# buwantaiji/FermiFlow

Hardware: AMD Instinct MI355X
Metric: walker-steps/sec (full VMC iteration: 100 MCMC steps + generate + E_loc + grad + Adam) (higher is better)
Workload: dtype f64

## Files before the change

fermiflow_amd/csrc/ff_cnf_adj.hip:

```cpp
#include "ff_common.h"
#include "ff_ode.h"
#include "ff_radial.h"

#ifdef FF_STAMPS
#define FF_STAMP(i) do { unsigned long long t_ = __builtin_amdgcn_s_memtime(); stamp_acc[i] += t_ - stamp_prev; stamp_prev = t_; } while (0)
#else
#define FF_STAMP(i) do { } while (0)
#endif

struct ff_adj_args {
  int64_t B;
  ff_net net;
  double ta, tb, rtol, atol;
  int max_steps;
  const double* z_in;
  const double* az_in;
  const double* ad_in;
  const double* w_e;
  const double* w_mean;
  const int32_t* w_index;
  double w_scale;
  double* gx_out;
  double* rows;
  double* trows;
  double* off_table;
  int32_t* stats;
  const double* h_init;
  double h_scale;
  int h_equal;
  double* h_out;
  int32_t* wcost;
  const int32_t* order;
  int unit0;
};

template <int N, int D, int MAXU>
__global__ void __launch_bounds__(FF_WAVE)
ff_ode_adj_kernel(ff_adj_args A) {
  using Gm = ff_geom<N, D>;
  constexpr int M = Gm::M, G = Gm::G, P = Gm::P, R = Gm::RA;
  constexpr int NV = 2;
  {
    const double* rt = A.net.radial_table;
    if (rt && rt[3] == 0.0 && rt[4] == 0.0 && *A.off_table == 0.0) return;
  }

  __shared__ ff_wtab s_w[2][FF_HPAD];
  __shared__ double s_z[G][M], s_kb[G][M], s_err[G][M], s_ad[G];
  __shared__ double s_rad[G][R], s_rinv[G][R], s_ca[G][R], s_cb[G][R];
  constexpr int CH = 8;
  __shared__ double s_ph[G][M][CH][3], s_hd[G][R][3];
  __shared__ int s_pa[R], s_pb[R], s_any;
  __shared__ double s_e2[64];

  __shared__ int s_st[4];
#include "ff_adj_direct_body.inc"
}

template <int N, int D>
struct ff_adj_smem {
  static constexpr int M = ff_geom<N, D>::M, G = ff_geom<N, D>::G, R = ff_geom<N, D>::RA, CH = 8;
  ff_wtab s_w[2][FF_HPAD];
  double s_z[G][M], s_kb[G][M], s_err[G][M], s_ad[G];
  double s_rad[G][R], s_rinv[G][R], s_ca[G][R], s_cb[G][R];
  double s_ph[G][M][CH][3], s_hd[G][R][3];
  double s_e2[64];
  int s_pa[R], s_pb[R], s_any, s_st[4];
};

template <int N, int D, int MAXU>
__global__ void __launch_bounds__(FF_WAVE, 4)
ff_ode_adj_lean_kernel(ff_adj_args A) {
  using Gm = ff_geom<N, D>;
  constexpr int M = Gm::M, G = Gm::G, P = Gm::P, R = Gm::RA;
  constexpr int NV = 2;
  {
    const double* rt = A.net.radial_table;
    if (rt && rt[3] == 0.0 && rt[4] == 0.0 && *A.off_table == 0.0) return;
  }
  FF_DYN_LDS(ff_adj_lean_lds);
  ff_adj_smem<N, D>& sm = *reinterpret_cast<ff_adj_smem<N, D>*>(ff_adj_lean_lds);
  auto& s_w = sm.s_w; auto& s_z = sm.s_z; auto& s_kb = sm.s_kb; auto& s_err = sm.s_err; auto& s_ad = sm.s_ad;
  auto& s_rad = sm.s_rad; auto& s_rinv = sm.s_rinv; auto& s_ca = sm.s_ca; auto& s_cb = sm.s_cb;
  constexpr int CH = ff_adj_smem<N, D>::CH;
  auto& s_ph = sm.s_ph; auto& s_hd = sm.s_hd; auto& s_pa = sm.s_pa; auto& s_pb = sm.s_pb; auto& s_any = sm.s_any;
  auto& s_e2 = sm.s_e2; auto& s_st = sm.s_st;
#include "ff_adj_direct_body.inc"
}

struct ff_rec { double dr, ca, cb; int j; };
#define FF_DEP_LROW (FF_DEP_ROW + 1)

FF_D void ff_row_add(double (*sW)[FF_DEP_NLDS][FF_DEP_LROW], double* __restrict__ ovf, int t, int j, const double* c, int nrow) {
  if (j < FF_DEP_NLDS) {
    double* row = &sW[t][j][0];
#pragma unroll
    for (int k = 0; k < 6; k++) atomicAdd(row + k, c[k]);
#pragma unroll
    for (int k0 = 6; k0 < FF_DEP_ROW; k0 += 2) {
      if (nrow > k0) { atomicAdd(row + k0, c[k0]); atomicAdd(row + k0 + 1, c[k0 + 1]); }
    }
  } else {
    double* row = ovf + ((size_t)t * FF_DEP_NTOT + j) * FF_DEP_ROW;
#pragma unroll
    for (int k = 0; k < FF_DEP_ROW; k++) atomicAdd(row + k, c[k]);
    int jo = j;
    FF_OPAQUE(jo);
  }
}

FF_D void ff_deposit(double (*sW)[FF_DEP_NLDS][FF_DEP_LROW], double* __restrict__ ovf, int t, const ff_rec& rc, double w, int nrow) {
  if (w == 0.0) return;
  double pk = 1.0, pm = 0.0, c[FF_DEP_ROW];
#pragma unroll
  for (int k = 0; k < FF_DEP_ROW; k++) {
    c[k] = w * fma(rc.ca, pk, rc.cb * pm);
    pm = pk;
    pk = pk * rc.dr * (1.0 / (k + 1));
  }
  ff_row_add(sW, ovf, t, rc.j, c, nrow);
}

FF_D void ff_deposit5(double (*sW)[FF_DEP_NLDS][FF_DEP_LROW], double* __restrict__ ovf, int t, const ff_rec& q0, const ff_rec& q2,
                      const ff_rec& q3, const ff_rec& q4, const ff_rec& q5, double hw, int nrow) {
  if (hw == 0.0) return;
  const ff_rec* rc[5] = {&q0, &q2, &q3, &q4, &q5};
  const double bw[5] = {hw * FF_B0, hw * FF_B2, hw * FF_B3, hw * FF_B4, hw * FF_B5};
  constexpr double HD = 1.0 / FF_DEP_INVH;
  double rm = 0.0;
#pragma unroll
  for (int e = 0; e < 5; e++) rm += fma((double)rc[e]->j, HD, rc[e]->dr);
  double jcf = rint(rm * (0.2 * FF_DEP_INVH));
  jcf = fmin(fmax(jcf, 0.0), (double)(FF_DEP_NTOT - 1));
  const int jC = (rm == rm) ? (int)jcf : 0;
  double acc[FF_DEP_ROW];
#pragma unroll
  for (int k = 0; k < FF_DEP_ROW; k++) acc[k] = 0.0;
#pragma unroll
  for (int e = 0; e < 5; e++) {
    const double dr = fma((double)(rc[e]->j - jC), HD, rc[e]->dr);
    if (fabs(dr) <= 1.5 * HD) {
      double pk = bw[e], pm = 0.0;
#pragma unroll
      for (int k = 0; k < FF_DEP_ROW; k++) {
        acc[k] += fma(rc[e]->ca, pk, rc[e]->cb * pm);
        pm = pk;
        pk = pk * dr * (1.0 / (k + 1));
      }
    } else {
      ff_deposit(sW, ovf, t, *rc[e], bw[e], nrow);
    }
  }
  ff_row_add(sW, ovf, t, jC, acc, nrow);
}

#ifndef FF_ADJ_WPS
#define FF_ADJ_WPS 1
#endif
#ifndef FF_ADJ_WPW
#define FF_ADJ_WPW 2
#endif
#ifndef FF_ADJ_G12
#define FF_ADJ_G12 3
#endif
constexpr int ff_adjtab_G(int n, int d) {
  const int M = n * d;
  if (M <= 0 || M > FF_WAVE) return 0;
  const int g = FF_WAVE / M > 16 ? 16 : FF_WAVE / M;
  if (M == 12) return FF_ADJ_G12;
  if (d == 2 && (n == 4 || n == 5 || n == 7 || n == 9 || n == 10 || n == 11)) {
    const int gr = FF_WAVE / (n * (n + 1) / 2);
    return gr < 1 ? 1 : (gr < g ? gr : g);
  }
  return g;
}
template <int N, int D> struct ff_adjtab_geom { static constexpr int G = ff_adjtab_G(N, D); };
static int adj_tab_G(int n, int d) { return ff_adjtab_G(n, d); }

template <int N, int D, int WPW>
__global__ void __launch_bounds__(FF_WAVE * WPW, WPW > 1 ? WPW : FF_ADJ_WPS)
ff_ode_adjtab_kernel(ff_adj_args A) {
  using Gm = ff_geom<N, D>;
  constexpr int M = Gm::M, G = ff_adjtab_geom<N, D>::G, P = Gm::P, R = Gm::RA;
  constexpr int NV = 2, NSLOT = (G * R + FF_WAVE - 1) / FF_WAVE;
#ifdef FF_PRIO_ADJTAB
  FF_SETPRIO();
#endif
  const double* __restrict__ rtab = A.net.radial_table;
  if (!(rtab && rtab[3] == 0.0 && rtab[4] == 0.0)) return;
  const int dep_nrow = FF_UNIFORM(rtab[5] >= 6.0 && rtab[5] <= (double)FF_DEP_ROW ? (int)rtab[5] : FF_DEP_ROW);

  __shared__ double s_z_[WPW][G][M], s_kb_[WPW][G][M], s_err_[WPW][G][M], s_ad_[WPW][G], s_hw_[WPW][G];
  constexpr int TROW = N * 3 * D + 1;
  __shared__ double s_T_[WPW][G][N][TROW];
  __shared__ double s_W[2][FF_DEP_NLDS][FF_DEP_LROW];
  __shared__ int s_pa[R], s_pb[R], s_any_[WPW];
  __shared__ int s_turn, s_done[2];

  const int wv = WPW > 1 ? (int)(threadIdx.x >> 6) : 0, lane = threadIdx.x & (FF_WAVE - 1);
  auto& s_z = s_z_[wv]; auto& s_kb = s_kb_[wv]; auto& s_err = s_err_[wv]; auto& s_ad = s_ad_[wv]; auto& s_hw = s_hw_[wv];
  auto& s_T = s_T_[wv]; int& s_any = s_any_[wv];
  const int g = lane / M, i = lane % M;
  const bool ingrp = g < G;
  const int gg = ingrp ? g : 0;
  const int ai = i / D, ci = i % D;
  for (int e = threadIdx.x; e < 2 * FF_DEP_NLDS * FF_DEP_LROW; e += FF_WAVE * WPW) (&s_W[0][0][0])[e] = 0.0;
  if (threadIdx.x == 0) {
    int p = 0;
    for (int a = 0; a < N; a++)
      for (int b = a + 1; b < N; b++) { s_pa[p] = a; s_pb[p] = b; p++; }
    for (int a = 0; a < N; a++) { if (P + a < R) { s_pa[P + a] = a; s_pb[P + a] = -1; } }
    s_turn = 0; s_done[0] = 0; s_done[1] = 0;
  }
  __syncthreads();
  const int He = A.net.He, Hm = A.net.Hm;
  const bool has_mu = Hm > 0;
  const int nrad = has_mu ? (P + N) : P;
  const double tab_inv_h = rtab[0], tab_h = rtab[1];
  const double rtol = A.rtol, atol = A.atol;
  int rq_id[NSLOT];
#pragma unroll
  for (int sl = 0; sl < NSLOT; sl++) {
    const int q = lane + sl * FF_WAVE;
    const bool act = q < G * nrad;
    const int qg = act ? q / nrad : 0, p = act ? q - qg * nrad : 0;
    rq_id[sl] = act ? (qg | (s_pa[p] << 4) | ((s_pb[p] < 0 ? 15 : s_pb[p]) << 8) | (p << 12)) : -1;
  }
  bool off_any = false;
  constexpr double NT = 2 * M;
  const int64_t ngroups = (A.B + G - 1) / G;
  __shared__ int s_st[4];
  if (threadIdx.x < 4) s_st[threadIdx.x] = 0;
  int my_turn = wv;
  double* const ovf = A.trows + (size_t)gridDim.x * 2 * FF_DEP_NLDS * FF_DEP_ROW;
#ifdef FF_STAMPS
  unsigned long long stamp_acc[9] = {0, 0, 0, 0, 0, 0, 0, 0, 0}, stamp_prev = __builtin_amdgcn_s_memtime();
#endif

  for (int64_t grp = (int64_t)blockIdx.x * WPW + wv; grp < ngroups; grp += (int64_t)gridDim.x * WPW) {
    const int64_t bq = grp * G + g;
    const bool valid = ingrp && bq < A.B;
    const int64_t b = ff_opt_load(A.order, valid, bq, A.z_in, (int32_t)bq);
    double y[NV], k0[NV] = {0.0, 0.0}, k1[NV] = {0.0, 0.0}, k2[NV] = {0.0, 0.0}, k3[NV] = {0.0, 0.0}, k4[NV] = {0.0, 0.0}, k5[NV] = {0.0, 0.0};
    y[0] = ff_opt_load(A.z_in, valid, b * M + i, A.z_in, 0.25 * (i + 1) + 0.125 * ((i * 7) % 5));
    {
      const bool ws = A.w_e != nullptr;
      const int wi = ff_opt_load(A.w_index, valid && ws, b, A.z_in, (int32_t)0);
      const double wb = (ff_opt_load(A.w_e, valid, b, A.z_in, 0.0) - ff_opt_load(A.w_mean, valid && ws, wi, A.z_in, 0.0)) * A.w_scale;
      const double az0 = ff_opt_load(A.az_in, valid, b * M + i, A.z_in, 0.0), ad0 = ff_opt_load(A.ad_in, valid, b, A.z_in, 0.0);
      y[1] = ws ? wb * az0 : az0;
      if (ingrp && i == 0) s_ad[g] = ws ? -wb : ad0;
    }
    ff_rec r0[NSLOT], r2[NSLOT], r3[NSLOT], r4[NSLOT], r5[NSLOT], r6[NSLOT];
    ff_stepper S;
    S.begin(A.ta, A.tb, valid);
    const double hwarm = ff_open_step(ff_opt_load(A.h_init, valid, A.h_scale < 0.0 ? 0 : b, A.z_in, 0.0) * fabs(A.h_scale), A.ta, A.tb, A.h_equal);
    const bool warm = hwarm > 0.0;
    double hmax_acc = 0.0;
    int s = -2, nev = 0;
    double h0v = 0.0, d1v = 0.0;

    auto group_sum = [&](double part) -> double {
      if (ingrp) s_err[g][i] = part;
      FF_WAVE_ORDER();
      double t = 0.0;
#pragma unroll
      for (int j = 0; j < M; j++) t += s_err[gg][j];
      FF_WAVE_ORDER();
      return t;
    };

    auto evaluate = [&](auto stage_tag) -> bool {
      constexpr int SG = decltype(stage_tag)::value;
      if constexpr (SG == FF_STAGE_DYN) FF_ASSUME(s <= 0);
      const int sv = SG == FF_STAGE_DYN ? s : SG;
      double in[NV];
      const double h = S.h;
      {
        const double hsel = (sv == -1) ? h0v * S.dir : h;
#pragma unroll
        for (int v = 0; v < NV; v++) in[v] = y[v];
        switch (sv) {
          case -1:
#pragma unroll
            for (int v = 0; v < NV; v++) in[v] = fma(hsel, k0[v], y[v]);
            break;
          case 1:
#pragma unroll
            for (int v = 0; v < NV; v++) in[v] = fma(hsel * FF_A10, k0[v], y[v]);
            break;
          case 2:
#pragma unroll
            for (int v = 0; v < NV; v++) in[v] = fma(hsel * FF_A21, k1[v], fma(hsel * FF_A20, k0[v], y[v]));
            break;
          case 3:
#pragma unroll
            for (int v = 0; v < NV; v++) in[v] = fma(hsel * FF_A32, k2[v], fma(hsel * FF_A31, k1[v], fma(hsel * FF_A30, k0[v], y[v])));
            break;
          case 4:
#pragma unroll
            for (int v = 0; v < NV; v++)
              in[v] = fma(hsel * FF_A43, k3[v], fma(hsel * FF_A42, k2[v], fma(hsel * FF_A41, k1[v], fma(hsel * FF_A40, k0[v], y[v]))));
            break;
          case 5:
#pragma unroll
            for (int v = 0; v < NV; v++)
              in[v] = fma(hsel * FF_A54, k4[v], fma(hsel * FF_A53, k3[v], fma(hsel * FF_A52, k2[v], fma(hsel * FF_A51, k1[v], fma(hsel * FF_A50, k0[v], y[v])))));
            break;
          case 6:
#pragma unroll
            for (int v = 0; v < NV; v++)
              in[v] = fma(hsel * FF_B5, k5[v], fma(hsel * FF_B4, k4[v], fma(hsel * FF_B3, k3[v], fma(hsel * FF_B2, k2[v], fma(hsel * FF_B0, k0[v], y[v])))));
            break;
          default: break;
        }
      }
      FF_STAMP(0);
      FF_WAVE_ORDER();
      if (ingrp) { s_z[g][i] = in[0]; s_kb[g][i] = in[1]; }
      FF_WAVE_ORDER();
      FF_STAMP(1);
      ff_rec cur[NSLOT];
      double rq_rho[NSLOT][D], rq_dl[NSLOT][D], rq_r[NSLOT], rq_ri[NSLOT], rq_T[NSLOT][3 + 5], rq_dr[NSLOT];
      bool rq_ok[NSLOT];
#pragma unroll
      for (int sl = 0; sl < NSLOT; sl++) {
        const int id = rq_id[sl];
        const bool act = id >= 0;
        const int qg = act ? (id & 15) : 0, a = act ? ((id >> 4) & 15) : 0, bq = act ? ((id >> 8) & 15) : 15;
        const bool pair = bq != 15;
        const int bb = pair ? bq : a;
        double r2 = 0.0;
#pragma unroll
        for (int c = 0; c < D; c++) {
          rq_rho[sl][c] = s_z[qg][a * D + c] - (pair ? s_z[qg][bb * D + c] : 0.0);
          rq_dl[sl][c] = s_kb[qg][a * D + c] - (pair ? s_kb[qg][bb * D + c] : 0.0);
          r2 = fma(rq_rho[sl][c], rq_rho[sl][c], r2);
        }
        ff_sqrt_rcp(r2, rq_r[sl], rq_ri[sl]);
        rq_dr[sl] = 0.0;
        rq_ok[sl] = ff_table_fetch<3>(rtab, tab_inv_h, tab_h, pair ? 0 : 1, rq_r[sl], rq_T[sl], rq_dr[sl]);
      }
#pragma unroll
      for (int sl = 0; sl < NSLOT; sl++) {
        const int id = rq_id[sl];
        cur[sl].j = 0; cur[sl].dr = 0.0; cur[sl].ca = 0.0; cur[sl].cb = 0.0;
        if (id >= 0) {
          const int qg = id & 15, a = (id >> 4) & 15, bq = (id >> 8) & 15;
          const bool pair = bq != 15;
          const int bb = pair ? bq : a;
          const double* rho = rq_rho[sl];
          const double* dl = rq_dl[sl];
          const double r = rq_r[sl], ri = rq_ri[sl], ad = s_ad[qg];
          double hd[3] = {0.0, 0.0, 0.0}, al = 0.0;
          if (rq_ok[sl]) ff_table_eval<3>(rq_T[sl], rq_dr[sl], hd);
#pragma unroll
          for (int c = 0; c < D; c++) al = fma(dl[c], rho[c], al);
          double jf = rint(r * FF_DEP_INVH);
          if ((!rq_ok[sl] || !(jf <= (double)(FF_DEP_NTOT - 1))) && (grp * G + qg) < A.B) off_any = true;
          jf = fmin(jf, (double)(FF_DEP_NTOT - 1));
          cur[sl].j = (r == r) ? (int)jf : 0;
          cur[sl].dr = fma(-jf, 1.0 / FF_DEP_INVH, r);
          cur[sl].ca = pair ? -(al - 2.0 * D * ad) : -(al - D * ad);
          cur[sl].cb = pair ? 2.0 * ad * r : ad * r;
          const double f0 = hd[0], f1 = hd[1], f2 = hd[2];
          const double F1 = f1 * (al * ri), gq = (pair ? 2.0 : 1.0) * fma(f2, r, (1.0 + D) * f1) * ri;
          double* Ta = &s_T[qg][a][bb * 3 * D];
#pragma unroll
          for (int c = 0; c < D; c++) {
            const double pv = f0 * rho[c], pw = fma(F1, rho[c], f0 * dl[c]), pg = gq * rho[c];
            Ta[c] = pv; Ta[D + c] = pw; Ta[2 * D + c] = pg;
          }
        }
      }
      FF_WAVE_ORDER();
      nev++;
      FF_STAMP(2);
      double out[NV];
      {
        double vi = 0.0, dvk = 0.0, gdi = 0.0;
#pragma unroll
        for (int j = 0; j < N; j++) {
          const bool use = has_mu || j != ai;
          const bool lower = j < ai;
          const double* T = lower ? &s_T[gg][j][ai * 3 * D + ci] : &s_T[gg][ai][j * 3 * D + ci];
          const double sg = lower ? -1.0 : 1.0;
          const double tv = T[0], tw = T[D], tg = T[2 * D];
          vi = fma(sg, use ? tv : 0.0, vi); dvk = fma(sg, use ? tw : 0.0, dvk); gdi = fma(sg, use ? tg : 0.0, gdi);
        }
        out[0] = vi;
        out[1] = fma(s_ad[gg], gdi, -dvk);
      }
      FF_STAMP(3);
      const int s_before = sv;
      if (sv == -2) {
#pragma unroll
        for (int v = 0; v < NV; v++) k0[v] = out[v];
#pragma unroll
        for (int sl = 0; sl < NSLOT; sl++) r0[sl] = cur[sl];
        double p0 = 0.0, p1 = 0.0;
#pragma unroll
        for (int v = 0; v < NV; v++) {
          const double isc = ff_rcp(fma(fabs(y[v]), rtol, atol));
          p0 = fma(y[v] * isc, y[v] * isc, p0);
          p1 = fma(k0[v] * isc, k0[v] * isc, p1);
        }
        const double d0 = sqrt(group_sum(p0) * (1.0 / NT));
        d1v = sqrt(group_sum(p1) * (1.0 / NT));
        h0v = S.h0(d0, d1v);
        s = -1;
        if (!ff_wave_or_w(&s_any, lane, (!S.done && !warm) ? 1 : 0)) {
          S.habs = fmin(hwarm, S.interval);
          S.plan();
          s = 1;
        }
      } else if (sv == -1) {
        double p2 = 0.0;
#pragma unroll
        for (int v = 0; v < NV; v++) {
          const double t = (out[v] - k0[v]) * ff_rcp(fma(fabs(y[v]), rtol, atol));
          p2 = fma(t, t, p2);
        }
        const double d2 = sqrt(group_sum(p2) * (1.0 / NT)) / h0v;
        S.init_habs(h0v, d1v, d2);
        if (warm) S.habs = fmin(hwarm, S.interval);
        S.plan();
        s = 1;
      } else if (sv == 0) {
#pragma unroll
        for (int v = 0; v < NV; v++) k0[v] = out[v];
#pragma unroll
        for (int sl = 0; sl < NSLOT; sl++) r0[sl] = cur[sl];
        s = 1;
      } else if (sv == 1) {
#pragma unroll
        for (int v = 0; v < NV; v++) k1[v] = out[v];
        s = 2;
      } else if (sv == 2) {
#pragma unroll
        for (int v = 0; v < NV; v++) k2[v] = out[v];
#pragma unroll
        for (int sl = 0; sl < NSLOT; sl++) r2[sl] = cur[sl];
        s = 3;
      } else if (sv == 3) {
#pragma unroll
        for (int v = 0; v < NV; v++) k3[v] = out[v];
#pragma unroll
        for (int sl = 0; sl < NSLOT; sl++) r3[sl] = cur[sl];
        s = 4;
      } else if (sv == 4) {
#pragma unroll
        for (int v = 0; v < NV; v++) k4[v] = out[v];
#pragma unroll
        for (int sl = 0; sl < NSLOT; sl++) r4[sl] = cur[sl];
        s = 5;
      } else if (sv == 5) {
#pragma unroll
        for (int v = 0; v < NV; v++) k5[v] = out[v];
#pragma unroll
        for (int sl = 0; sl < NSLOT; sl++) r5[sl] = cur[sl];
        s = 6;
      } else {
#pragma unroll
        for (int sl = 0; sl < NSLOT; sl++) r6[sl] = cur[sl];
        double pe = 0.0;
#pragma unroll
        for (int v = 0; v < NV; v++) {
          const double e = h * (FF_E0 * k0[v] + FF_E2 * k2[v] + FF_E3 * k3[v] + FF_E4 * k4[v] + FF_E5 * k5[v] + FF_E6 * out[v]);
          const double t = e * ff_rcp(fma(fmax(fabs(y[v]), fabs(in[v])), rtol, atol));
          pe = fma(t, t, pe);
        }
        const double err = sqrt(group_sum(pe) * (1.0 / NT));
        const bool was_active = !S.done;
        const bool acc = S.decide(err, A.max_steps);
        if (acc) hmax_acc = fmax(hmax_acc, fabs(h));
        if (acc) {
#pragma unroll
          for (int v = 0; v < NV; v++) { y[v] = in[v]; k0[v] = out[v]; }
        }
        if (ingrp && i == 0) s_hw[g] = acc ? h : 0.0;
        FF_WAVE_ORDER();
#ifndef FF_ADJ_NOTICKET
        if constexpr (WPW > 1) {
          while (__hip_atomic_load(&s_turn, __ATOMIC_RELAXED, __HIP_MEMORY_SCOPE_WORKGROUP) != my_turn &&
                 !__hip_atomic_load(&s_done[1 - wv], __ATOMIC_RELAXED, __HIP_MEMORY_SCOPE_WORKGROUP))
            __builtin_amdgcn_s_sleep(1);
          FF_WAVE_SYNC();
        }
#endif
#pragma unroll
        for (int sl = 0; sl < NSLOT; sl++) {
          if (rq_id[sl] >= 0) {
            const int qg = rq_id[sl] & 15;
            const int t = ((rq_id[sl] >> 8) & 15) != 15 ? 0 : 1;
            const double hw = s_hw[qg];
#ifndef FF_ADJ_NODEP
            ff_deposit5(s_W, ovf, t, r0[sl], r2[sl], r3[sl], r4[sl], r5[sl], hw, dep_nrow);
#endif
            if (hw != 0.0) r0[sl] = r6[sl];
          }
        }
        if constexpr (WPW > 1) {
          FF_WAVE_SYNC();
          if (lane == 0) __hip_atomic_store(&s_turn, my_turn + 1, __ATOMIC_RELAXED, __HIP_MEMORY_SCOPE_WORKGROUP);
          my_turn += 2;
        }
        S.plan();
        const int any = ff_wave_or_w(&s_any, lane, S.done ? 0 : ((was_active && !acc) ? 3 : 1));
        s = (any & 2) ? 0 : 1;
        if (!any) { FF_STAMP(5); return true; }
      }
      if (s_before == 6) FF_STAMP(5); else FF_STAMP(4);
      return false;
    };
#pragma unroll 1
    for (;;) {
#pragma unroll 1
      while (s <= 0) evaluate(ff_stage_c<FF_STAGE_DYN>{});
      evaluate(ff_stage_c<1>{});
      evaluate(ff_stage_c<2>{});
      evaluate(ff_stage_c<3>{});
      evaluate(ff_stage_c<4>{});
      evaluate(ff_stage_c<5>{});
      if (evaluate(ff_stage_c<6>{})) break;
    }
    if (valid) {
      const double bad = S.fail ? __builtin_nan("") : 0.0;
      if (A.gx_out) A.gx_out[b * M + i] = y[1] + bad;
      if (i == 0) {
        if (S.fail) atomicAdd(&s_W[0][0][0], bad);
        if (A.h_out) A.h_out[b] = hmax_acc > 0.0 ? hmax_acc : hwarm;
        if (A.wcost) A.wcost[b] = S.nacc + S.nrej;
        if (A.stats) { atomicAdd(&s_st[0], nev); atomicMax(&s_st[1], S.nacc); atomicAdd(&s_st[2], S.nrej); if (S.fail) atomicMax(&s_st[3], 1); }
      }
    }
    FF_WAVE_ORDER();
  }
#ifdef FF_STAMPS
  if (A.stats && lane == 0)
    for (int q = 0; q < 9; q++) atomicAdd((unsigned long long*)(A.stats + 8) + q, stamp_acc[q]);
#endif
  if (off_any) *A.off_table = 1.0;
  if constexpr (WPW > 1) {
    FF_WAVE_SYNC();
    if (lane == 0) __hip_atomic_store(&s_done[wv], 1, __ATOMIC_RELAXED, __HIP_MEMORY_SCOPE_WORKGROUP);
  }
  __syncthreads();
  {
    double* row = A.trows + (size_t)blockIdx.x * 2 * FF_DEP_NLDS * FF_DEP_ROW;
    for (int e = threadIdx.x; e < 2 * FF_DEP_NLDS * FF_DEP_ROW; e += FF_WAVE * WPW) row[e] = (&s_W[0][0][0])[(e / FF_DEP_ROW) * FF_DEP_LROW + e % FF_DEP_ROW];
  }
  __syncthreads();
  if (A.stats && threadIdx.x == 0 && (s_st[0] || s_st[3])) {
    atomicAdd(&A.stats[0], s_st[0]);
    atomicMax(&A.stats[1], s_st[1]);
    atomicAdd(&A.stats[2], s_st[2]);
    if (s_st[3]) atomicMax(&A.stats[3], 1);
  }
}

extern bool ff_wide_forced();
extern int ff_wide_supported(int n, int d);
#include "ff_adj_wide.h"

#ifndef FF_DEPR_EX
#define FF_DEPR_EX 16
#define FF_DEPR_TY 16
#endif
__global__ void __launch_bounds__(FF_DEPR_EX * FF_DEPR_TY)
ff_adj_reduce_kernel(ff_net net, const double* __restrict__ off_table, int nrows, int P, const double* __restrict__ prow,
                     double* __restrict__ out, int nblocks, const double* __restrict__ rows, double* __restrict__ wtot) {
  FF_SETPRIO();
  const double* rtab = net.radial_table;
  const bool tab_served = rtab && rtab[3] == 0.0 && rtab[4] == 0.0 && *off_table == 0.0;
  if ((int)blockIdx.x < P) {
    if (tab_served) return;
    __shared__ double smr[FF_DEPR_EX * FF_DEPR_TY];
    const int k = blockIdx.x;
    double sr = 0.0;
    for (int r = threadIdx.x; r < nrows; r += blockDim.x) sr += prow[(int64_t)r * P + k];
    smr[threadIdx.x] = sr;
    __syncthreads();
    for (int w = blockDim.x / 2; w > 0; w >>= 1) {
      if ((int)threadIdx.x < w) smr[threadIdx.x] += smr[threadIdx.x + w];
      __syncthreads();
    }
    if (threadIdx.x == 0) out[k] = smr[0];
    return;
  }
  if (!tab_served || rows == nullptr) return;
  const int bid = (int)blockIdx.x - P;
  __shared__ double sm[FF_DEPR_TY][FF_DEPR_EX + 1];
  const int tx = threadIdx.x % FF_DEPR_EX, ty = threadIdx.x / FF_DEPR_EX;
  const int e = bid * FF_DEPR_EX + tx;
  constexpr int NE = 2 * FF_DEP_NLDS * FF_DEP_ROW;
  double sp[8] = {0.0, 0.0, 0.0, 0.0, 0.0, 0.0, 0.0, 0.0};
  if (e < NE) {
    int b = ty;
    for (; b + 7 * FF_DEPR_TY < nblocks; b += 8 * FF_DEPR_TY) {
#pragma unroll
      for (int u = 0; u < 8; u++) sp[u] += rows[(size_t)(b + u * FF_DEPR_TY) * NE + e];
    }
#pragma unroll
    for (int u = 0; u < 8; u++)
      if (b + u * FF_DEPR_TY < nblocks) sp[u] += rows[(size_t)(b + u * FF_DEPR_TY) * NE + e];
  }
  sm[ty][tx] = ((sp[0] + sp[1]) + (sp[2] + sp[3])) + ((sp[4] + sp[5]) + (sp[6] + sp[7]));
  __syncthreads();
  for (int w = FF_DEPR_TY / 2; w > 0; w >>= 1) {
    if (ty < w) sm[ty][tx] += sm[ty + w][tx];
    __syncthreads();
  }
  if (ty == 0 && e < NE) {
    const int t = e / (FF_DEP_NLDS * FF_DEP_ROW), rem = e - t * FF_DEP_NLDS * FF_DEP_ROW;
    wtot[(size_t)t * FF_DEP_NTOT * FF_DEP_ROW + rem] = sm[0][tx];
  }
}

__constant__ double FF_SIGPOLY_MEM[13][14] = FF_SIGPOLY_INIT;
__global__ void __launch_bounds__(256)
ff_dep_contract_kernel(ff_net net, const double* __restrict__ off_table, const double* __restrict__ wtot, double* __restrict__ grad) {
  FF_SETPRIO();
  const double* rtab = net.radial_table;
  if (!(rtab && rtab[3] == 0.0 && rtab[4] == 0.0 && *off_table == 0.0)) return;
  __shared__ double sm[3][256];
  __shared__ double s_W[FF_DEP_NTOT * FF_DEP_ROW];
  __shared__ double s_P[13 * 14];
  const int t = blockIdx.x < (unsigned)net.He ? 0 : 1, hu = t ? blockIdx.x - net.He : blockIdx.x;
  const int H = t ? net.Hm : net.He;
  const double w1 = (t ? net.mw1 : net.ew1)[hu], b1 = (t ? net.mb1 : net.eb1)[hu], w2 = (t ? net.mw2 : net.ew2)[hu];
  {
    const double* Wt = wtot + (size_t)t * FF_DEP_NTOT * FF_DEP_ROW;
    for (int e = threadIdx.x; e < FF_DEP_NTOT * FF_DEP_ROW; e += blockDim.x) s_W[e] = Wt[e];
    for (int e = threadIdx.x; e < 13 * 14; e += blockDim.x) s_P[e] = (&FF_SIGPOLY_MEM[0][0])[e];
  }
  __syncthreads();
  double gw1 = 0.0, gb1 = 0.0, gw2 = 0.0;
  for (int j = threadIdx.x; j < FF_DEP_NTOT; j += blockDim.x) {
    const double rj = (double)j * (1.0 / FF_DEP_INVH);
    const double sg = ff_sigmoid(fma(w1, rj, b1));
    const double* W = &s_W[j * FF_DEP_ROW];
    {
      bool any = false;
#pragma unroll
      for (int k = 0; k < FF_DEP_ROW; k++) any = any || (W[k] != 0.0);
      if (!any) continue;
    }
    double wk = 1.0, wkm = 0.0, prev = 0.0;
#pragma unroll 1
    for (int n = 0; n <= FF_DEP_ROW; n++) {
      double p = s_P[n * 14 + n + 1];
#pragma unroll 1
      for (int c = n; c >= 1; c--) p = fma(p, sg, s_P[n * 14 + c]);
      const double cur = p * sg;
      if (n >= 1) {
        const double Wk = W[n - 1];
        gw2 = fma(Wk, wk * prev, gw2);
        gb1 = fma(Wk, w2 * wk * cur, gb1);
        gw1 = fma(Wk, w2 * fma(wkm, prev, wk * rj * cur), gw1);
        wkm = (double)n * wk;
        wk *= w1;
      }
      prev = cur;
    }
  }
  sm[0][threadIdx.x] = gw1; sm[1][threadIdx.x] = gb1; sm[2][threadIdx.x] = gw2;
  __syncthreads();
  for (int w = blockDim.x / 2; w > 0; w >>= 1) {
    if ((int)threadIdx.x < w)
      for (int c = 0; c < 3; c++) sm[c][threadIdx.x] += sm[c][threadIdx.x + w];
    __syncthreads();
  }
  if (threadIdx.x == 0) {
    double* gout = grad + (t ? 3 * net.He : 0);
    gout[hu] = sm[0][0]; gout[H + hu] = sm[1][0]; gout[2 * H + hu] = sm[2][0];
  }
}

__global__ void __launch_bounds__(256) ff_zero_kernel(double* __restrict__ p, size_t n) {
  for (size_t k = blockIdx.x * (size_t)blockDim.x + threadIdx.x; k < n; k += (size_t)gridDim.x * blockDim.x) p[k] = 0.0;
}

extern void ff_set_error(const char* msg);
#define FF_CHECK(cond, code, msg) do { if (!(cond)) { ff_set_error(msg); return code; } } while (0)
#define FF_LAUNCH_CHECK() do { hipError_t e_ = hipGetLastError(); if (e_ != hipSuccess) { ff_set_error(hipGetErrorString(e_)); return FF_ELAUNCH; } } while (0)

#include <stdlib.h>

static int adj_G(int n, int d) { int M = n * d; return M > 0 && M <= FF_WAVE ? (FF_WAVE / M > 16 ? 16 : FF_WAVE / M) : 0; }
static int64_t adj_default_blocks() {
  static int64_t n = 0;
  if (n == 0) {
    int dev = 0, cus = 0;
    if (hipGetDevice(&dev) != hipSuccess || hipDeviceGetAttribute(&cus, hipDeviceAttributeMultiprocessorCount, dev) != hipSuccess || cus <= 0)
      cus = 256;
    n = 4 * (int64_t)cus;
  }
  return n;
}

static unsigned adj_grid(int64_t B, int G) {
  int64_t ngroups = (B + G - 1) / G;
  const int64_t cap = adj_default_blocks();
  return (unsigned)(ngroups < cap ? ngroups : cap);
}

template <int N, int D>
static void launch_adj(void* stream, const ff_adj_args& a_in) {
  constexpr int M = ff_geom<N, D>::M;
  constexpr int MU_64 = (64 + M - 1) / M > 16 ? 16 : (64 + M - 1) / M, MU_50 = (50 + M - 1) / M > 16 ? 16 : (50 + M - 1) / M;
  const int hmax = a_in.net.He > a_in.net.Hm ? a_in.net.He : a_in.net.Hm;
  ff_adj_args a = a_in;
  const bool lean = a_in.net.radial_table != nullptr;
  const size_t lds = sizeof(ff_adj_smem<N, D>);
  if (MU_50 < MU_64 && hmax <= MU_50 * M) {
    a.unit0 = 0;
    if (lean) FF_LAUNCH_LDS((ff_ode_adj_lean_kernel<N, D, MU_50>), adj_grid(a.B, ff_geom<N, D>::G), FF_WAVE, lds, stream, a);
    else FF_LAUNCH((ff_ode_adj_kernel<N, D, MU_50>), adj_grid(a.B, ff_geom<N, D>::G), FF_WAVE, stream, a);
  } else {
    for (int u0 = 0; u0 < hmax; u0 += MU_64 * M) {
      a.unit0 = u0;
      if (lean) FF_LAUNCH_LDS((ff_ode_adj_lean_kernel<N, D, MU_64>), adj_grid(a.B, ff_geom<N, D>::G), FF_WAVE, lds, stream, a);
      else FF_LAUNCH((ff_ode_adj_kernel<N, D, MU_64>), adj_grid(a.B, ff_geom<N, D>::G), FF_WAVE, stream, a);
    }
  }
}

__global__ void __launch_bounds__(256) ff_open_steps_kernel(int64_t B, const double* __restrict__ h_init, double scale, double ta, double tb,
                                                            double* __restrict__ out) {
  const int64_t b = (int64_t)blockIdx.x * blockDim.x + threadIdx.x;
  if (b < B) out[b] = ff_open_step(h_init[b] * scale, ta, tb, 1);
}

extern "C" {

static size_t adj_table_doubles(int64_t B, int Gtab) {
  return (size_t)adj_grid(B, Gtab) * 2 * FF_DEP_NLDS * FF_DEP_ROW + (size_t)2 * FF_DEP_NTOT * FF_DEP_ROW;
}

static size_t adj_direct_doubles(int64_t B, int G, int He, int Hm) { return (size_t)adj_grid(B, G) * G * (size_t)(3 * He + 3 * Hm); }

static bool adj_is_wide(int n, int d) {
  const bool narrow = (d == 2 && n >= 1 && n <= 12) || (d == 3 && n >= 2 && n <= 4);
  return ff_wide_supported(n, d) && (!narrow || ff_wide_forced());
}

static size_t adj_ws_doubles(bool wide, int64_t B, int n, int d, int He, int Hm) {
  if (wide) return ff_wide_supported(n, d) ? adj_direct_doubles(B, 1, He, Hm) + adj_table_doubles(B, 1) + 1 + (size_t)B : 0;
  const bool narrow = (d == 2 && n >= 1 && n <= 12) || (d == 3 && n >= 2 && n <= 4);
  const int G = adj_G(n, d);
  return (narrow && G) ? adj_direct_doubles(B, G, He, Hm) + adj_table_doubles(B, adj_tab_G(n, d) * FF_ADJ_WPW) + 1 : 0;
}

size_t ff_cnf_adjoint_workspace_bytes(int64_t B, int n, int d, int He, int Hm) {
  if (B <= 0) return 0;
  const size_t a = adj_ws_doubles(false, B, n, d, He, Hm), b = adj_ws_doubles(true, B, n, d, He, Hm);
  return sizeof(double) * (a > b ? a : b);
}

static int adjoint_impl(void* stream, int64_t B, int n, int d, const ff_net* net, const ff_ode* ode, const double* z_t0,
                        const double* a_z, const double* a_d, const double* w_e, const double* w_mean, const int32_t* w_index,
                        double w_scale, double* grad_x, double* grad_params, void* workspace, int32_t* stats);

int ff_cnf_adjoint(void* stream, int64_t B, int n, int d, const ff_net* net, const ff_ode* ode, const double* z_t0,
                   const double* a_z, const double* a_d, double* grad_x, double* grad_params, void* workspace,
                   int32_t* stats) {
  FF_CHECK(B == 0 || a_d, FF_EINVAL, "ff_cnf_adjoint: null pointer");
  return adjoint_impl(stream, B, n, d, net, ode, z_t0, a_z, a_d, nullptr, nullptr, nullptr, 0.0, grad_x, grad_params, workspace, stats);
}

int ff_cnf_adjoint_energy(void* stream, int64_t B, int n, int d, const ff_net* net, const ff_ode* ode, const double* z_t0,
                          const double* glogp0, const double* eloc, const double* e_mean, const int32_t* mean_index, double scale,
                          double* grad_x, double* grad_params, void* workspace, int32_t* stats) {
  FF_CHECK(B == 0 || (eloc && e_mean), FF_EINVAL, "ff_cnf_adjoint_energy: null pointer");
  return adjoint_impl(stream, B, n, d, net, ode, z_t0, glogp0, nullptr, eloc, e_mean, mean_index, scale, grad_x, grad_params, workspace,
                      stats);
}

static int adjoint_impl(void* stream, int64_t B, int n, int d, const ff_net* net, const ff_ode* ode, const double* z_t0,
                        const double* a_z, const double* a_d, const double* w_e, const double* w_mean, const int32_t* w_index,
                        double w_scale, double* grad_x, double* grad_params, void* workspace, int32_t* stats) {
  FF_CHECK(B >= 0 && n > 0 && d > 0 && net && ode && grad_params, FF_EINVAL, "ff_cnf_adjoint: bad argument");
  FF_CHECK(net->He > 0 && net->ew1 && net->eb1 && net->ew2 && (net->Hm == 0 || (net->mw1 && net->mb1 && net->mw2)), FF_EINVAL,
           "ff_cnf_adjoint: bad net");
  FF_CHECK(net->He <= FF_HMAX && net->Hm <= FF_HMAX, FF_EUNSUPPORTED, "ff_cnf_adjoint: hidden width > 256");
  FF_CHECK(ode->rtol > 0 && ode->atol > 0, FF_EINVAL, "ff_cnf_adjoint: tolerances must be positive");
  const int P = 3 * net->He + 3 * net->Hm;
  if (B == 0) {
    if (hipMemsetAsync(grad_params, 0, sizeof(double) * P, (hipStream_t)stream) != hipSuccess) return FF_ELAUNCH;
    return FF_OK;
  }
  FF_CHECK(z_t0 && a_z && workspace, FF_EINVAL, "ff_cnf_adjoint: null pointer");
  ff_adj_args a = {};
  a.B = B; a.net = *net; a.ta = ode->t0; a.tb = ode->t1; a.rtol = ode->rtol; a.atol = ode->atol;
  a.max_steps = ode->max_steps > 0 ? ode->max_steps : 10000;
  a.wcost = ode->walker_cost; a.order = ode->walker_order;
  a.h_init = ode->walker_h_init; a.h_scale = ode->walker_h_uniform ? -fabs(ode->walker_h_scale) : fabs(ode->walker_h_scale); a.h_out = ode->walker_h_out; a.h_equal = ode->walker_h_equal;
  a.z_in = z_t0; a.az_in = a_z; a.ad_in = a_d; a.w_e = w_e; a.w_mean = w_mean; a.w_index = w_index; a.w_scale = w_scale; a.gx_out = grad_x; a.rows = (double*)workspace; a.stats = stats;
  const bool wide = adj_is_wide(n, d);
  {
    const int Gq = wide ? 1 : adj_G(n, d);
    if (Gq == 0) { ff_set_error("ff_cnf_adjoint: n*d > 64"); return FF_EUNSUPPORTED; }
    a.trows = a.rows + adj_direct_doubles(B, Gq, net->He, net->Hm);
    a.off_table = a.trows + adj_table_doubles(B, wide ? 1 : adj_tab_G(n, d) * FF_ADJ_WPW);
  }
  if (wide) {
    if (hipMemsetAsync(workspace, 0, sizeof(double) * adj_ws_doubles(wide, B, n, d, net->He, net->Hm), (hipStream_t)stream) != hipSuccess) return FF_ELAUNCH;
  } else {
    double* wt = a.off_table - (size_t)2 * FF_DEP_NTOT * FF_DEP_ROW;
    FF_LAUNCH(ff_zero_kernel, 48, 256, stream, wt, (size_t)2 * FF_DEP_NTOT * FF_DEP_ROW + 1);
  }
  int G = 0;
  if (wide && a.h_equal && a.h_init) {
    const int64_t nh = a.h_scale < 0.0 ? 1 : B;
    double* hs = a.off_table + 1;
    FF_LAUNCH(ff_open_steps_kernel, (unsigned)((nh + 255) / 256), 256, stream, nh, a.h_init, fabs(a.h_scale), a.ta, a.tb, hs);
    a.h_init = hs; a.h_scale = a.h_scale < 0.0 ? -1.0 : 1.0; a.h_equal = 0;
  }
  if (wide) {
    const int nr = n * (n + 1) / 2, Wv = nr <= 128 ? 2 : 4, nq = (nr + 64 * Wv - 1) / (64 * Wv);
    const unsigned grid = adj_grid(a.B, 1);
#define FF_WA(D_, W_, Q_) if (d == D_ && Wv == W_ && nq == Q_) { if (net->radial_table) FF_LAUNCH((ff_wide_adjtab_kernel<D_, W_, Q_>), grid, FF_WAVE * W_, stream, a, n); \
                                                                  FF_LAUNCH((ff_wide_adj_kernel<D_, W_, Q_>), grid, FF_WAVE * W_, stream, a, n); G = 1; }
    FF_WA(2, 2, 1) FF_WA(2, 4, 1) FF_WA(2, 4, 2) FF_WA(3, 2, 1) FF_WA(3, 4, 1) FF_WA(3, 4, 2)
#undef FF_WA
  } else
#define FF_ND(N_, D_) if (n == N_ && d == D_) { if (net->radial_table) FF_LAUNCH((ff_ode_adjtab_kernel<N_, D_, FF_ADJ_WPW>), adj_grid(a.B, ff_adjtab_geom<N_, D_>::G * FF_ADJ_WPW), FF_WAVE * FF_ADJ_WPW, stream, a); launch_adj<N_, D_>(stream, a); G = ff_geom<N_, D_>::G; }
  FF_ND(6, 2) else FF_ND(3, 2) else FF_ND(12, 2) else FF_ND(2, 2) else FF_ND(4, 2) else FF_ND(5, 2) else FF_ND(8, 2) else FF_ND(10, 2)
  else FF_ND(1, 2) else FF_ND(7, 2) else FF_ND(9, 2) else FF_ND(11, 2) else FF_ND(2, 3) else FF_ND(3, 3) else FF_ND(4, 3)
#undef FF_ND
  if (G == 0) {
    ff_set_error("fused CNF kernels serve n <= 24 particles with n*d <= 60 in d = 2, 3");
    return FF_EUNSUPPORTED;
  }
  FF_LAUNCH_CHECK();
  if (ode->after_main_event && hipEventRecord((hipEvent_t)ode->after_main_event, (hipStream_t)stream) != hipSuccess) {
    ff_set_error("ff_cnf_adjoint: hipEventRecord(after_main_event) failed");
    return FF_ELAUNCH;
  }
  const int nblk = (int)adj_grid(B, G);
  {
    const int ntab = (int)adj_grid(B, wide ? 1 : adj_tab_G(n, d) * FF_ADJ_WPW);
    double* wtot = a.trows + (size_t)ntab * 2 * FF_DEP_NLDS * FF_DEP_ROW;
    const unsigned ndep = net->radial_table ? (unsigned)((2 * FF_DEP_NLDS * FF_DEP_ROW + FF_DEPR_EX - 1) / FF_DEPR_EX) : 0u;
    FF_LAUNCH(ff_adj_reduce_kernel, (unsigned)P + ndep, FF_DEPR_EX * FF_DEPR_TY, stream, *net, (const double*)a.off_table, nblk * G, P,
              (const double*)a.rows, grad_params, ntab, (const double*)(net->radial_table ? a.trows : nullptr), wtot);
    FF_LAUNCH_CHECK();
  }
  if (net->radial_table) {
    const int ntab = (int)adj_grid(B, wide ? 1 : adj_tab_G(n, d) * FF_ADJ_WPW);
    double* wtot = a.trows + (size_t)ntab * 2 * FF_DEP_NLDS * FF_DEP_ROW;
    FF_LAUNCH(ff_dep_contract_kernel, (unsigned)(net->He + net->Hm), FF_RBLOCK(256), stream, *net, (const double*)a.off_table,
              (const double*)wtot, grad_params);
    FF_LAUNCH_CHECK();
  }
  return FF_OK;
}

}
```

Baseline: 5.677 billion.

## Replace LDS atomic row deposits with wave-elected serialized rounds

Deposits into the shared LDS table no longer use one atomicAdd per coefficient. Lanes that target the same row are ranked through an LDS bitmask election, and the rows are then committed in rank-ordered rounds with plain read-modify-write. The row length is specialized at compile time (6/8/10/full) through a switch on dep_nrow. For a single slot, the accumulation and ranking are hoisted ahead of the inter-wave ticket wait, and far-away records are deposited in separate ballot-guarded passes. This trades atomic contention for extra wave-order barriers and ballot loops. It also reuses the s_T scratch area as election storage, which is only safe if s_T is dead at that point.

```diff
diff --git a/fermiflow_amd/csrc/ff_cnf_adj.hip b/fermiflow_amd/csrc/ff_cnf_adj.hip
--- a/fermiflow_amd/csrc/ff_cnf_adj.hip
+++ b/fermiflow_amd/csrc/ff_cnf_adj.hip
@@ -90,40 +90,85 @@
 
 struct ff_rec { double dr, ca, cb; int j; };
 #define FF_DEP_LROW (FF_DEP_ROW + 1)
-
-FF_D void ff_row_add(double (*sW)[FF_DEP_NLDS][FF_DEP_LROW], double* __restrict__ ovf, int t, int j, const double* c, int nrow) {
-  if (j < FF_DEP_NLDS) {
+#define FF_DEP_NELECT (2 * 2 * FF_DEP_NLDS)
+typedef int __attribute__((may_alias)) ff_elect_t;
+
+FF_D int ff_row_rank(ff_elect_t* s_el, int lane, bool part, int key) {
+  const int slot = part ? 2 * key : 0;
+  if (part) { s_el[slot] = 0; s_el[slot + 1] = 0; }
+  FF_WAVE_ORDER();
+  if (part) atomicOr((int*)&s_el[slot + (lane >> 5)], (int)(1u << (lane & 31)));
+  FF_WAVE_ORDER();
+  const unsigned lo = part ? (unsigned)s_el[slot] : 0u, hi = part ? (unsigned)s_el[slot + 1] : 0u;
+  FF_WAVE_ORDER();
+  const unsigned long long members = ((unsigned long long)hi << 32) | lo;
+  return part ? __popcll(members & ((1ull << lane) - 1ull)) : -1;
+}
+
+template <int NR, bool ROUNDS>
+FF_D void ff_rows_commit(double (*sW)[FF_DEP_NLDS][FF_DEP_LROW], double* __restrict__ ovf, int t, int j, bool act, int rank, const double* c) {
+  if constexpr (ROUNDS) {
+#ifdef FF_ADJ_HYBRID
+    if (rank == 0) {
+      double* row = &sW[t][j][0];
+      double v[NR];
+#pragma unroll
+      for (int k = 0; k < NR; k++) v[k] = row[k];
+#pragma unroll
+      for (int k = 0; k < NR; k++) row[k] = v[k] + c[k];
+    }
+    FF_WAVE_ORDER();
+    if (rank > 0) {
+      double* row = &sW[t][j][0];
+#pragma unroll
+      for (int k = 0; k < NR; k++) atomicAdd(row + k, c[k]);
+    }
+#else
+    for (int r = 0; ff_wave_ballot(rank >= r); r++) {
+      if (rank == r) {
+        double* row = &sW[t][j][0];
+        double v[NR];
+#pragma unroll
+        for (int k = 0; k < NR; k++) v[k] = row[k];
+#pragma unroll
+        for (int k = 0; k < NR; k++) row[k] = v[k] + c[k];
+      }
+      FF_WAVE_ORDER();
+    }
+#endif
+  } else if (act && j < FF_DEP_NLDS) {
     double* row = &sW[t][j][0];
 #pragma unroll
-    for (int k = 0; k < 6; k++) atomicAdd(row + k, c[k]);
-#pragma unroll
-    for (int k0 = 6; k0 < FF_DEP_ROW; k0 += 2) {
-      if (nrow > k0) { atomicAdd(row + k0, c[k0]); atomicAdd(row + k0 + 1, c[k0 + 1]); }
-    }
-  } else {
+    for (int k = 0; k < NR; k++) atomicAdd(row + k, c[k]);
+  }
+  if (act && j >= FF_DEP_NLDS) {
     double* row = ovf + ((size_t)t * FF_DEP_NTOT + j) * FF_DEP_ROW;
 #pragma unroll
-    for (int k = 0; k < FF_DEP_ROW; k++) atomicAdd(row + k, c[k]);
+    for (int k = 0; k < NR; k++) atomicAdd(row + k, c[k]);
     int jo = j;
     FF_OPAQUE(jo);
   }
 }
 
-FF_D void ff_deposit(double (*sW)[FF_DEP_NLDS][FF_DEP_LROW], double* __restrict__ ovf, int t, const ff_rec& rc, double w, int nrow) {
-  if (w == 0.0) return;
-  double pk = 1.0, pm = 0.0, c[FF_DEP_ROW];
-#pragma unroll
-  for (int k = 0; k < FF_DEP_ROW; k++) {
+template <int NR, bool ROUNDS>
+FF_D void ff_deposit(double (*sW)[FF_DEP_NLDS][FF_DEP_LROW], double* __restrict__ ovf, ff_elect_t* s_el, int lane, int t, const ff_rec& rc,
+                     double w, bool act) {
+  act = act && w != 0.0;
+  double pk = 1.0, pm = 0.0, c[NR];
+#pragma unroll
+  for (int k = 0; k < NR; k++) {
     c[k] = w * fma(rc.ca, pk, rc.cb * pm);
     pm = pk;
     pk = pk * rc.dr * (1.0 / (k + 1));
   }
-  ff_row_add(sW, ovf, t, rc.j, c, nrow);
-}
-
-FF_D void ff_deposit5(double (*sW)[FF_DEP_NLDS][FF_DEP_LROW], double* __restrict__ ovf, int t, const ff_rec& q0, const ff_rec& q2,
-                      const ff_rec& q3, const ff_rec& q4, const ff_rec& q5, double hw, int nrow) {
-  if (hw == 0.0) return;
+  int rank = -1;
+  if constexpr (ROUNDS) rank = ff_row_rank(s_el, lane, act && rc.j < FF_DEP_NLDS, t * FF_DEP_NLDS + rc.j);
+  ff_rows_commit<NR, ROUNDS>(sW, ovf, t, rc.j, act, rank, c);
+}
+
+template <int NR>
+FF_D void ff_deposit5_row(const ff_rec& q0, const ff_rec& q2, const ff_rec& q3, const ff_rec& q4, const ff_rec& q5, double hw, int& jC,
+                          double* acc, int& far) {
   const ff_rec* rc[5] = {&q0, &q2, &q3, &q4, &q5};
   const double bw[5] = {hw * FF_B0, hw * FF_B2, hw * FF_B3, hw * FF_B4, hw * FF_B5};
   constexpr double HD = 1.0 / FF_DEP_INVH;
@@ -132,26 +177,43 @@
   for (int e = 0; e < 5; e++) rm += fma((double)rc[e]->j, HD, rc[e]->dr);
   double jcf = rint(rm * (0.2 * FF_DEP_INVH));
   jcf = fmin(fmax(jcf, 0.0), (double)(FF_DEP_NTOT - 1));
-  const int jC = (rm == rm) ? (int)jcf : 0;
-  double acc[FF_DEP_ROW];
-#pragma unroll
-  for (int k = 0; k < FF_DEP_ROW; k++) acc[k] = 0.0;
+  jC = (rm == rm) ? (int)jcf : 0;
+  far = 0;
+#pragma unroll
+  for (int k = 0; k < NR; k++) acc[k] = 0.0;
 #pragma unroll
   for (int e = 0; e < 5; e++) {
     const double dr = fma((double)(rc[e]->j - jC), HD, rc[e]->dr);
     if (fabs(dr) <= 1.5 * HD) {
       double pk = bw[e], pm = 0.0;
 #pragma unroll
-      for (int k = 0; k < FF_DEP_ROW; k++) {
+      for (int k = 0; k < NR; k++) {
         acc[k] += fma(rc[e]->ca, pk, rc[e]->cb * pm);
         pm = pk;
         pk = pk * dr * (1.0 / (k + 1));
       }
     } else {
-      ff_deposit(sW, ovf, t, *rc[e], bw[e], nrow);
-    }
-  }
-  ff_row_add(sW, ovf, t, jC, acc, nrow);
+      far |= 1 << e;
+    }
+  }
+}
+
+template <int NR, bool ROUNDS>
+FF_D void ff_deposit_far(double (*sW)[FF_DEP_NLDS][FF_DEP_LROW], double* __restrict__ ovf, ff_elect_t* s_el, int lane, int t,
+                         const ff_rec& q0, const ff_rec& q2, const ff_rec& q3, const ff_rec& q4, const ff_rec& q5, double hw, int far) {
+  if (!ff_wave_ballot(far != 0)) return;
+  const ff_rec* rc[5] = {&q0, &q2, &q3, &q4, &q5};
+  const double bw[5] = {hw * FF_B0, hw * FF_B2, hw * FF_B3, hw * FF_B4, hw * FF_B5};
+#pragma unroll 1
+  for (int e = 0; e < 5; e++) {
+    if (!ff_wave_ballot(((far >> e) & 1) != 0)) continue;
+    ff_rec q = *rc[0];
+    double w = bw[0];
+#pragma unroll
+    for (int u = 1; u < 5; u++)
+      if (e == u) { q = *rc[u]; w = bw[u]; }
+    ff_deposit<NR, ROUNDS>(sW, ovf, s_el, lane, t, q, w, ((far >> e) & 1) != 0);
+  }
 }
 
 #ifndef FF_ADJ_WPS
@@ -193,6 +255,11 @@
   __shared__ double s_z_[WPW][G][M], s_kb_[WPW][G][M], s_err_[WPW][G][M], s_ad_[WPW][G], s_hw_[WPW][G];
   constexpr int TROW = N * 3 * D + 1;
   __shared__ double s_T_[WPW][G][N][TROW];
+#ifdef FF_ADJ_ATOMIC_ROWS
+  constexpr bool DEP_ROUNDS = false;
+#else
+  constexpr bool DEP_ROUNDS = sizeof(double) * G * N * TROW >= sizeof(int) * FF_DEP_NELECT;
+#endif
   __shared__ double s_W[2][FF_DEP_NLDS][FF_DEP_LROW];
   __shared__ int s_pa[R], s_pb[R], s_any_[WPW];
   __shared__ int s_turn, s_done[2];
@@ -480,25 +547,51 @@
         }
         if (ingrp && i == 0) s_hw[g] = acc ? h : 0.0;
         FF_WAVE_ORDER();
+        auto deposit_phase = [&](auto nr_tag) {
+          constexpr int NR = decltype(nr_tag)::value;
+          constexpr bool PRE = NSLOT == 1;
+          ff_elect_t* const s_el = reinterpret_cast<ff_elect_t*>(&s_T[0][0][0]);
+          int d_t[NSLOT], d_j[NSLOT], d_far[NSLOT], d_rank[NSLOT];
+          bool d_act[NSLOT];
+          double d_hw[NSLOT], d_acc[NSLOT][NR];
+          auto prepare = [&](int sl) {
+            d_act[sl] = rq_id[sl] >= 0;
+            const int qg = d_act[sl] ? (rq_id[sl] & 15) : 0;
+            d_t[sl] = ((rq_id[sl] >> 8) & 15) != 15 ? 0 : 1;
+            d_hw[sl] = s_hw[qg];
+            d_act[sl] = d_act[sl] && d_hw[sl] != 0.0;
+            d_far[sl] = 0; d_rank[sl] = -1; d_j[sl] = 0;
+#ifndef FF_ADJ_NODEP
+            ff_deposit5_row<NR>(r0[sl], r2[sl], r3[sl], r4[sl], r5[sl], d_hw[sl], d_j[sl], d_acc[sl], d_far[sl]);
+            if (!d_act[sl]) d_far[sl] = 0;
+            if constexpr (DEP_ROUNDS)
+              d_rank[sl] = ff_row_rank(s_el, lane, d_act[sl] && d_j[sl] < FF_DEP_NLDS, d_t[sl] * FF_DEP_NLDS + d_j[sl]);
+#endif
+          };
+          if constexpr (PRE) prepare(0);
 #ifndef FF_ADJ_NOTICKET
-        if constexpr (WPW > 1) {
-          while (__hip_atomic_load(&s_turn, __ATOMIC_RELAXED, __HIP_MEMORY_SCOPE_WORKGROUP) != my_turn &&
-                 !__hip_atomic_load(&s_done[1 - wv], __ATOMIC_RELAXED, __HIP_MEMORY_SCOPE_WORKGROUP))
-            __builtin_amdgcn_s_sleep(1);
-          FF_WAVE_SYNC();
-        }
-#endif
-#pragma unroll
-        for (int sl = 0; sl < NSLOT; sl++) {
-          if (rq_id[sl] >= 0) {
-            const int qg = rq_id[sl] & 15;
-            const int t = ((rq_id[sl] >> 8) & 15) != 15 ? 0 : 1;
-            const double hw = s_hw[qg];
+          if constexpr (WPW > 1) {
+            while (__hip_atomic_load(&s_turn, __ATOMIC_RELAXED, __HIP_MEMORY_SCOPE_WORKGROUP) != my_turn &&
+                   !__hip_atomic_load(&s_done[1 - wv], __ATOMIC_RELAXED, __HIP_MEMORY_SCOPE_WORKGROUP))
+              __builtin_amdgcn_s_sleep(1);
+            FF_WAVE_SYNC();
+          }
+#endif
+#pragma unroll
+          for (int sl = 0; sl < NSLOT; sl++) {
+            if constexpr (!PRE) prepare(sl);
 #ifndef FF_ADJ_NODEP
-            ff_deposit5(s_W, ovf, t, r0[sl], r2[sl], r3[sl], r4[sl], r5[sl], hw, dep_nrow);
-#endif
-            if (hw != 0.0) r0[sl] = r6[sl];
+            ff_rows_commit<NR, DEP_ROUNDS>(s_W, ovf, d_t[sl], d_j[sl], d_act[sl], d_rank[sl], d_acc[sl]);
+            ff_deposit_far<NR, DEP_ROUNDS>(s_W, ovf, s_el, lane, d_t[sl], r0[sl], r2[sl], r3[sl], r4[sl], r5[sl], d_hw[sl], d_far[sl]);
+#endif
+            if (d_act[sl]) r0[sl] = r6[sl];
           }
+        };
+        switch (dep_nrow) {
+          case 6: deposit_phase(ff_stage_c<6>{}); break;
+          case 8: deposit_phase(ff_stage_c<8>{}); break;
+          case 10: deposit_phase(ff_stage_c<10>{}); break;
+          default: deposit_phase(ff_stage_c<FF_DEP_ROW>{}); break;
         }
         if constexpr (WPW > 1) {
           FF_WAVE_SYNC();
```

Result: slower. 5.515 billion (median of 2 runs) (-2.8%).
